# ssilverman16/particle_col_image_segmentation

Measured on AMD Instinct MI355X. Metric: Mpixels/sec segmented (5-ch 1024x1024 TIFF), ROI mask IoU=1.0, higher is better.
Workload: dtype f32 planes / u8 class maps / int32 labels / f64 ROI sums; 1 GPU; BASELINE config 2: batch of 64 frames 1024x1024x5 float32 per GPU, full kernel chain, inputs resident in HBM; frames_per_gpu=64, height=1024, width=1024, planes=5, parallelism=frames x1, launch=one hipGraph replay per step, 4 in flight, tie_fallback_frames_last_step=0, reference_nan_frames_rank0=0

## Files before the change

### particle_col_image_segmentation_amd/csrc/watershed.hip

```cpp
#include <algorithm>
#include <atomic>
#include <climits>
#include <mutex>
#include <type_traits>

#include "common.h"

namespace pcseg {

constexpr int WS_T = 64;
constexpr int WS_S = WS_T + 2;
constexpr int WS_P = 67;
constexpr int WS_N = WS_S * WS_P;
constexpr unsigned WS_INF = 0xFFFFFFFFu;
constexpr int WS_CNT0 = 32, WS_CNT_STRIDE = 32, WS_CHANGED_INTS = WS_CNT0 + 16 * WS_CNT_STRIDE;

__device__ __forceinline__ unsigned ws_key(float f)
{
    if (f == 0.0f) f = 0.0f;
    unsigned u = __float_as_uint(f);
    u = (u & 0x80000000u) ? ~u : (u | 0x80000000u);
    return u == WS_INF ? WS_INF - 1 : u;
}

__global__ void __launch_bounds__(256) ws_init_kernel(const float *__restrict__ img, int64_t frame_stride,
                                                       const int *__restrict__ markers, const uint8_t *__restrict__ mask,
                                                       unsigned *__restrict__ val, unsigned *__restrict__ L,
                                                       int *__restrict__ out, int64_t n, int64_t total)
{
    int64_t i = (int64_t)blockIdx.x * blockDim.x + threadIdx.x;
    if (i >= total) return;
    bool m = mask[i] != 0;
    unsigned v = m ? ws_key(img[(i / n) * frame_stride + (i % n)]) : WS_INF;
    int mk = m ? markers[i] : 0;
    val[i] = v;
    L[i] = mk != 0 ? v : WS_INF;
    out[i] = mk;
}

template <typename T>
__device__ __forceinline__ void ws_store_tile(const T *s, T *__restrict__ g, int r0, int c0, int H, int W)
{
    for (int i = threadIdx.x; i < WS_T * WS_T; i += blockDim.x) {
        int lr = i / WS_T, lc = i % WS_T;
        int r = r0 + lr, c = c0 + lc;
        if (r < H && c < W) g[rowoff(r, W) + c] = s[(lr + 1) * WS_P + lc + 1];
    }
}

template <typename T>
__device__ __forceinline__ void ws_mark_changed_edges(const T *s, const T *__restrict__ g, uint8_t *dirty_out,
                                                      int b, int tx, int ty, int tilesX, int tilesY, int r0, int c0, int H, int W)
{
    if (threadIdx.x >= 256) return;
    const int e = threadIdx.x >> 6, j = threadIdx.x & 63;
    const int lr = e == 0 ? 1 : (e == 1 ? WS_T : j + 1);
    const int lc = e == 2 ? 1 : (e == 3 ? WS_T : j + 1);
    const int r = r0 + lr - 1, c = c0 + lc - 1;
    bool ch = false;
    if (r < H && c < W) ch = s[lr * WS_P + lc] != g[rowoff(r, W) + c];
    if (__any(ch) && j == 0) {
        uint8_t *d = dirty_out + (int64_t)b * tilesX * tilesY;
        if (e == 0 && ty > 0) d[(ty - 1) * tilesX + tx] = 1;
        else if (e == 1 && ty + 1 < tilesY) d[(ty + 1) * tilesX + tx] = 1;
        else if (e == 2 && tx > 0) d[ty * tilesX + tx - 1] = 1;
        else if (e == 3 && tx + 1 < tilesX) d[ty * tilesX + tx + 1] = 1;
    }
}

template <int T>
struct RelaxGeom {
    static_assert(T == 64, "relaxation tiles are 64 pixels wide: one wave per sweep quadrant");
    static constexpr int S = T + 2;
    static constexpr int P = T + 4;
    static constexpr int PAD = 8;
    static constexpr int N = S * P + 2 * PAD;
    static constexpr int THREADS = 4 * 64;
    static constexpr int HE = T / 2;
    static constexpr size_t LDS_BYTES = sizeof(uint2) * N;
};

template <int DR, int DC, int P>
__device__ __forceinline__ bool ws_quadrant_sweep(uint2 *sLV, int lane)
{
    unsigned *sLw = reinterpret_cast<unsigned *>(sLV);
    typedef unsigned u2v __attribute__((ext_vector_type(2)));
    unsigned long long diff = 0;
    {
        constexpr int fr = DR > 0 ? 1 : WS_T, hr = DR > 0 ? 0 : WS_T + 1;
        const uint2 c = sLV[fr * P + 1 + lane];
        const unsigned h = sLV[hr * P + 1 + lane].x;
        const unsigned nw = min(c.x, max(c.y, h));
        atomicMin(&sLw[2 * (fr * P + 1 + lane)], nw);
        diff |= __ballot(nw != c.x);
    }
    const int lr = DR > 0 ? lane + 1 : WS_T - lane;
    const uint2 *row = sLV + lr * P;
    const unsigned halo = row[DC > 0 ? 0 : WS_T + 1].x;
    const int u0 = (0 - lane) & 63;
    unsigned left = row[DC > 0 ? u0 : WS_T + 1 - u0].x;
    const int un = (0 - (lane + 1)) & 63;
    unsigned prev = row[DC > 0 ? 1 + un : WS_T - un].x;
    const unsigned a0 = (unsigned)(uintptr_t)(row + (DC > 0 ? 1 : WS_T));
#pragma unroll 1
    for (int j0 = 0; j0 < WS_T; j0 += 8) {
        const int ub = (u0 + j0) & 63;
        const unsigned base_a = DC > 0 ? a0 + 8u * (unsigned)ub : a0 - 8u * (unsigned)ub - 56u;
        const unsigned base_b = DC > 0 ? base_a - 512u : base_a + 512u;
        unsigned ba[8];
        u2v t[8];
#define PCSEG_DS_READ(k)                                                                                                   \
        {                                                                                                                      \
            const unsigned long long wrapped = (((1ull << (k)) - 1ull) << 1) << j0;                \
            asm("v_cndmask_b32_e64 %0, %1, %2, %3" : "=v"(ba[k]) : "v"(base_a), "v"(base_b), "s"(wrapped));                     \
            asm volatile("ds_read_b64 %0, %1 offset:%2" : "=v"(t[k]) : "v"(ba[k]), "n"(DC > 0 ? 8 * (k) : 8 * (7 - (k))));     \
        }
        PCSEG_DS_READ(0) PCSEG_DS_READ(1) PCSEG_DS_READ(2) PCSEG_DS_READ(3)
        PCSEG_DS_READ(4) PCSEG_DS_READ(5) PCSEG_DS_READ(6) PCSEG_DS_READ(7)
#undef PCSEG_DS_READ
        asm volatile("s_waitcnt lgkmcnt(0)" : "+v"(t[0]), "+v"(t[1]), "+v"(t[2]), "+v"(t[3]), "+v"(t[4]), "+v"(t[5]), "+v"(t[6]), "+v"(t[7]));
        unsigned wr[8];
        unsigned long long batch_diff = 0;
#pragma unroll
        for (int k = 0; k < 8; ++k) {
            const unsigned up = (unsigned)__builtin_amdgcn_update_dpp((int)WS_INF, (int)prev, 0x138, 0xF, 0xF, false);
            const unsigned long long at0 = (1ull << k) << j0;
            unsigned lf;
            asm("v_cndmask_b32_e64 %0, %1, %2, %3" : "=v"(lf) : "v"(left), "v"(halo), "s"(at0));
            const unsigned cur = t[k].x, v = t[k].y;
            const unsigned m = min(up, lf);
            const unsigned cand = min(max(v, m), max(min(v, m), cur));
            wr[k] = cand;
            batch_diff |= __ballot(cur != cand);
            left = cand;
            prev = cand;
        }
        if (batch_diff != 0) {
#define PCSEG_DS_MIN(k)                                                                                                             \
            asm volatile("ds_min_u32 %0, %1 offset:%2" : : "v"(ba[k]), "v"(wr[k]), "n"(DC > 0 ? 8 * (k) : 8 * (7 - (k))) : "memory");
            PCSEG_DS_MIN(0) PCSEG_DS_MIN(1) PCSEG_DS_MIN(2) PCSEG_DS_MIN(3)
            PCSEG_DS_MIN(4) PCSEG_DS_MIN(5) PCSEG_DS_MIN(6) PCSEG_DS_MIN(7)
#undef PCSEG_DS_MIN
            diff |= batch_diff;
        }
    }
    return diff != 0;
}

struct WsInputs {
    const float *img;
    int64_t frame_stride;
    const int *markers;
    const uint8_t *mask;
    int *out;
    bool vec;
};

struct WsTiling {
    int off;
    int nx, ny;
};

template <int T>
__device__ __forceinline__ void ws_relax_tile(uint2 *sLV, const WsInputs &in, const bool FIRST, unsigned *__restrict__ val,
                                              unsigned *__restrict__ L, uint8_t *__restrict__ dirty_in,
                                              uint8_t *__restrict__ dirty_out, int *__restrict__ any_changed, int H, int W,
                                              const WsTiling &cur, const WsTiling &nxt, int max_iter, int tx, int ty, int b,
                                              int *__restrict__ list_out = nullptr, int *__restrict__ count_out = nullptr)
{
    using G = RelaxGeom<T>;
    constexpr int S = G::S, P = G::P, NT = G::THREADS, QW = T / 4;
    const int tid = threadIdx.x;
    if (!FIRST) {
        uint8_t *mark = dirty_in + ((int64_t)b * cur.ny + ty) * cur.nx + tx;
        if (!*mark) return;
        __syncthreads();
        if (tid == 0) *mark = 0;
    }
    if (tid == 0) atomicAdd(any_changed + WS_CNT0 + WS_CNT_STRIDE * ((tx + 5 * ty + 3 * b) & 15), 1);
    const int r0 = ty * T - cur.off, c0 = tx * T - cur.off;
    const int64_t fbase = (int64_t)b * H * W;
    auto initial = [&](int r, int c) -> uint2 {
        const int64_t g = fbase + rowoff(r, W) + c;
        if (!in.mask[g]) return make_uint2(WS_INF, WS_INF);
        const unsigned v = ws_key(in.img[(int64_t)b * in.frame_stride + rowoff(r, W) + c]);
        return make_uint2(in.markers[g] != 0 ? v : WS_INF, v);
    };
    if (in.vec) {
        constexpr int QUADS = S * QW, TRIPS = (QUADS + NT - 1) / NT;
        const float *img_f = in.img + (int64_t)b * in.frame_stride;
        const bool halo_thread = tid < 2 * S;
        const int h_lr = tid >> 1, h_lc = (tid & 1) ? S - 1 : 0;
        const int h_r = r0 + h_lr - 1, h_c = c0 + h_lc - 1;
        const bool h_in = halo_thread && h_r >= 0 && h_r < H && h_c >= 0 && h_c < W;
        const int64_t h_p = rowoff(min(max(h_r, 0), H - 1), W) + min(max(h_c, 0), W - 1);
        if (FIRST) {
            float4 f4[TRIPS];
            int4 m4[TRIPS];
            unsigned k4[TRIPS];
#pragma unroll
            for (int t = 0; t < TRIPS; ++t) {
                const int idx = min(tid + NT * t, QUADS - 1);
                const int lr = idx / QW, q = idx % QW;
                const int64_t p = rowoff(min(max(r0 + lr - 1, 0), H - 1), W) + min(max(c0 + 4 * q, 0), W - 4);
                f4[t] = *reinterpret_cast<const float4 *>(img_f + p);
                m4[t] = *reinterpret_cast<const int4 *>(in.markers + fbase + p);
                k4[t] = *reinterpret_cast<const unsigned *>(in.mask + fbase + p);
            }
            const float hf = img_f[h_p];
            const int hm = in.markers[fbase + h_p];
            const uint8_t hk = in.mask[fbase + h_p];
#pragma unroll
            for (int t = 0; t < TRIPS; ++t) {
                const int idx = tid + NT * t;
                if (idx < QUADS) {
                    const int lr = idx / QW, q = idx % QW;
                    const int r = r0 + lr - 1, c = c0 + 4 * q;
                    const bool inside = r >= 0 && r < H && c >= 0 && c < W;
                    const float fv[4] = {f4[t].x, f4[t].y, f4[t].z, f4[t].w};
                    const int mv[4] = {m4[t].x, m4[t].y, m4[t].z, m4[t].w};
                    unsigned key[4];
                    int lab[4];
#pragma unroll
                    for (int j = 0; j < 4; ++j) {
                        const bool msk = inside && ((k4[t] >> (8 * j)) & 255u) != 0;
                        key[j] = msk ? ws_key(fv[j]) : WS_INF;
                        lab[j] = msk ? mv[j] : 0;
                        sLV[lr * P + 1 + 4 * q + j] = make_uint2(lab[j] != 0 ? key[j] : WS_INF, key[j]);
                    }
                    if (inside && lr >= 1 && lr <= T) {
                        const int64_t g = fbase + rowoff(r, W) + c;
                        *reinterpret_cast<uint4 *>(val + g) = make_uint4(key[0], key[1], key[2], key[3]);
                        *reinterpret_cast<int4 *>(in.out + g) = make_int4(lab[0], lab[1], lab[2], lab[3]);
                    }
                }
            }
            if (halo_thread) {
                const bool msk = h_in && hk != 0;
                const unsigned key = msk ? ws_key(hf) : WS_INF;
                sLV[h_lr * P + h_lc] = make_uint2(msk && hm != 0 ? key : WS_INF, key);
            }
        } else {
            uint4 l4[TRIPS], v4[TRIPS];
#pragma unroll
            for (int t = 0; t < TRIPS; ++t) {
                const int idx = min(tid + NT * t, QUADS - 1);
                const int lr = idx / QW, q = idx % QW;
                const int64_t p = fbase + rowoff(min(max(r0 + lr - 1, 0), H - 1), W) + min(max(c0 + 4 * q, 0), W - 4);
                l4[t] = *reinterpret_cast<const uint4 *>(L + p);
                v4[t] = *reinterpret_cast<const uint4 *>(val + p);
            }
            const unsigned hl = L[fbase + h_p], hv = val[fbase + h_p];
#pragma unroll
            for (int t = 0; t < TRIPS; ++t) {
                const int idx = tid + NT * t;
                if (idx < QUADS) {
                    const int lr = idx / QW, q = idx % QW;
                    const int r = r0 + lr - 1, c = c0 + 4 * q;
                    const bool inside = r >= 0 && r < H && c >= 0 && c < W;
                    uint2 *dst = sLV + lr * P + 1 + 4 * q;
                    dst[0] = inside ? make_uint2(l4[t].x, v4[t].x) : make_uint2(WS_INF, WS_INF);
                    dst[1] = inside ? make_uint2(l4[t].y, v4[t].y) : make_uint2(WS_INF, WS_INF);
                    dst[2] = inside ? make_uint2(l4[t].z, v4[t].z) : make_uint2(WS_INF, WS_INF);
                    dst[3] = inside ? make_uint2(l4[t].w, v4[t].w) : make_uint2(WS_INF, WS_INF);
                }
            }
            if (halo_thread) sLV[h_lr * P + h_lc] = h_in ? make_uint2(hl, hv) : make_uint2(WS_INF, WS_INF);
        }
    } else
    for (int i = tid; i < S * S; i += NT) {
        int lr = i / S, lc = i % S;
        int r = r0 + lr - 1, c = c0 + lc - 1;
        uint2 lv = make_uint2(WS_INF, WS_INF);
        if (r >= 0 && r < H && c >= 0 && c < W) {
            if (FIRST) {
                lv = initial(r, c);
                if (lr >= 1 && lr <= T && lc >= 1 && lc <= T) {
                    const int64_t g = fbase + rowoff(r, W) + c;
                    val[g] = lv.y;
                    in.out[g] = lv.y != WS_INF ? in.markers[g] : 0;
                }
            } else {
                lv.x = L[fbase + rowoff(r, W) + c];
                lv.y = val[fbase + rowoff(r, W) + c];
            }
        }
        sLV[lr * P + lc] = lv;
    }
    __syncthreads();
    const bool rim_thread = tid < 8 * G::HE;
    const int e = tid / G::HE, ej = tid % G::HE;
    const int qy = e < 4 ? (e >> 1) : (e & 1), qx = e < 4 ? (e & 1) : ((e >> 1) & 1);
    const int rim_lr = e < 4 ? (qy ? T : 1) : qy * G::HE + ej + 1;
    const int rim_lc = e < 4 ? qx * G::HE + ej + 1 : (qx ? T : 1);
    const unsigned rim_before = rim_thread ? sLV[rim_lr * P + rim_lc].x : 0u;
    const int dir = (tid >> 6) & 3, lane = tid & 63;
    bool changed_any = false;
    bool capped = true;
    for (int iter = 0; iter < max_iter; ++iter) {
        bool changed;
        if (dir == 0) changed = ws_quadrant_sweep<1, 1, P>(sLV, lane);
        else if (dir == 1) changed = ws_quadrant_sweep<1, -1, P>(sLV, lane);
        else if (dir == 2) changed = ws_quadrant_sweep<-1, 1, P>(sLV, lane);
        else changed = ws_quadrant_sweep<-1, -1, P>(sLV, lane);
        if (!__syncthreads_or(changed)) { capped = false; break; }
        changed_any = true;
    }
    if (!FIRST && !changed_any) return;
    if (changed_any) {
        const int r = r0 + rim_lr - 1, c = c0 + rim_lc - 1;
        bool ch = rim_thread && capped;
        if (rim_thread && !capped && r >= 0 && r < H && c >= 0 && c < W) ch = sLV[rim_lr * P + rim_lc].x != rim_before;
        const unsigned long long mine = ((1ull << G::HE) - 1ull) << ((tid & 63) / G::HE * G::HE);
        const unsigned long long edge_changed = __ballot(ch) & mine;
        if (rim_thread && edge_changed && ej == 0) {
            const int oy = (r0 + qy * G::HE + nxt.off) / T, ox = (c0 + qx * G::HE + nxt.off) / T;
            if (oy >= 0 && oy < nxt.ny && ox >= 0 && ox < nxt.nx) {
                const int64_t m = ((int64_t)b * nxt.ny + oy) * nxt.nx + ox;
                if (list_out) {
                    const unsigned bit = 1u << (8 * (int)(m & 3));
                    const unsigned old = atomicOr(reinterpret_cast<unsigned *>(dirty_out + (m & ~(int64_t)3)), bit);
                    if (!(old & bit)) list_out[atomicAdd(count_out, 1)] = (int)m;
                } else {
                    dirty_out[m] = 1;
                }
            }
        }
    }
    __syncthreads();
    if (in.vec) {
#pragma unroll
        for (int t = 0; t < T * QW / NT; ++t) {
            const int idx = tid + NT * t, lr = idx / QW, q = idx % QW;
            const int r = r0 + lr, c = c0 + 4 * q;
            const uint2 *src = sLV + (lr + 1) * P + 1 + 4 * q;
            if (r >= 0 && r < H && c >= 0 && c < W)
                *reinterpret_cast<uint4 *>(L + fbase + rowoff(r, W) + c) = make_uint4(src[0].x, src[1].x, src[2].x, src[3].x);
        }
        return;
    }
    for (int i = tid; i < T * T; i += NT) {
        int lr = i / T, lc = i % T;
        int r = r0 + lr, c = c0 + lc;
        if (r >= 0 && r < H && c >= 0 && c < W) L[fbase + rowoff(r, W) + c] = sLV[(lr + 1) * P + lc + 1].x;
    }
}

template <int T>
__global__ void __launch_bounds__(RelaxGeom<T>::THREADS) ws_relax_kernel(WsInputs in, const bool FIRST, unsigned *__restrict__ val,
                                                                         unsigned *__restrict__ L, uint8_t *__restrict__ dirty_in,
                                                                         uint8_t *__restrict__ dirty_out, int *__restrict__ any_changed,
                                                                         int H, int W, WsTiling cur, WsTiling nxt, int max_iter,
                                                                         int *__restrict__ list_out, int *__restrict__ count_out)
{
    extern __shared__ __attribute__((aligned(16))) uint2 relax_lds[];
    const TileIndex t = xcd_tile_index();
    ws_relax_tile<T>(relax_lds + RelaxGeom<T>::PAD, in, FIRST, val, L, dirty_in, dirty_out, any_changed, H, W, cur, nxt, max_iter, t.x, t.y,
                     t.z, list_out, count_out);
}

constexpr int WS_LIST_FROM = 4, WS_LIST_GRID = 1024;

template <int T>
__global__ void __launch_bounds__(RelaxGeom<T>::THREADS) ws_relax_list_kernel(WsInputs in, unsigned *__restrict__ val, unsigned *__restrict__ L,
                                                                              uint8_t *__restrict__ dirty_in, uint8_t *__restrict__ dirty_out,
                                                                              int *__restrict__ any_changed, int H, int W, WsTiling cur,
                                                                              WsTiling nxt, int max_iter, const int *__restrict__ list_in,
                                                                              const int *__restrict__ count_in, int *__restrict__ list_out,
                                                                              int *__restrict__ count_out)
{
    extern __shared__ __attribute__((aligned(16))) uint2 relax_lds[];
    const int n = *count_in, per_frame = cur.nx * cur.ny;
    for (int i = blockIdx.x; i < n; i += gridDim.x) {
        const int m = list_in[i], b = m / per_frame, t = m % per_frame;
        ws_relax_tile<T>(relax_lds + RelaxGeom<T>::PAD, in, false, val, L, dirty_in, dirty_out, any_changed, H, W, cur, nxt, max_iter,
                         t % cur.nx, t / cur.nx, b, list_out, count_out);
        __syncthreads();
    }
}

constexpr int WS_TAIL_LIST = 1024;

template <int T>
__global__ void __launch_bounds__(RelaxGeom<T>::THREADS) ws_relax_tail_kernel(WsInputs in, unsigned *__restrict__ val,
                                                                              unsigned *__restrict__ L, uint8_t *__restrict__ dirtyA,
                                                                              uint8_t *__restrict__ dirtyB, int *__restrict__ any_changed,
                                                                              int *__restrict__ not_converged, int *__restrict__ exact_flags,
                                                                              int H, int W, WsTiling t0, WsTiling t1, int first_round,
                                                                              int max_rounds)
{
    extern __shared__ __attribute__((aligned(16))) uint2 relax_lds[];
    __shared__ int tail_list[WS_TAIL_LIST];
    __shared__ int tail_count;
    const int b = blockIdx.x;
    uint8_t *din = dirtyA, *dout = dirtyB;
    for (int round = first_round;; ++round) {
        const WsTiling cur = (round & 1) ? t1 : t0, nxt = (round & 1) ? t0 : t1;
        const int ntiles = cur.nx * cur.ny;
        const uint8_t *marks = din + (int64_t)b * ntiles;
        if (threadIdx.x == 0) tail_count = 0;
        __syncthreads();
        for (int t = threadIdx.x; t < ntiles; t += RelaxGeom<T>::THREADS)
            if (marks[t] != 0) {
                const int k = atomicAdd(&tail_count, 1);
                if (k < WS_TAIL_LIST) tail_list[k] = t;
            }
        __syncthreads();
        const int marked = tail_count;
        if (marked == 0) return;
        if (round - first_round >= max_rounds) {
            if (threadIdx.x == 0) { *not_converged = 1; exact_flags[b] = 1; }
            return;
        }
        const int walk = marked <= WS_TAIL_LIST ? marked : ntiles;
        for (int k = 0; k < walk; ++k) {
            const int t = marked <= WS_TAIL_LIST ? tail_list[k] : k;
            ws_relax_tile<T>(relax_lds + RelaxGeom<T>::PAD, in, false, val, L, din, dout, any_changed, H, W, cur, nxt, 100000, t % cur.nx,
                             t / cur.nx, b);
            __syncthreads();
        }
        uint8_t *tmp = din; din = dout; dout = tmp;
    }
}


constexpr int WS_LIST_SPAN = 8;
template <typename Body>
__device__ __forceinline__ void ws_for_frames(const int *frame_list, int grid_index, int grid_size, Body &&body)
{
    if (!frame_list) {
        body(grid_index);
        return;
    }
    const int n = frame_list[-1];
    for (int gi = grid_index; gi < n; gi += grid_size) body(frame_list[gi]);
}
static inline int ws_frame_span(const int *frame_list, int B) { return frame_list ? (B < WS_LIST_SPAN ? B : WS_LIST_SPAN) : B; }

__device__ __forceinline__ bool ws_active(const uint8_t *active, int b, int r, int c, int tilesX, int tilesY)
{
    return active == nullptr || active[((int64_t)b * tilesY + r / WS_T) * tilesX + c / WS_T] != 0;
}

struct WsTileList {
    const int *list;
    int ntpf, tilesX;
};
constexpr int WS_TILE_GRID = 512;

template <typename Body>
__device__ __forceinline__ void ws_for_tiles(const WsTileList &tl, Body &&body)
{
    const int n = tl.list[-1];
    for (int i = blockIdx.x; i < n; i += gridDim.x) {
        const int e = tl.list[i], b = e / tl.ntpf, t = e % tl.ntpf;
        body(b, t % tl.tilesX, t / tl.tilesX);
    }
}

__global__ void __launch_bounds__(256) ws_list_tiles_kernel(const int *__restrict__ frame_list, const uint8_t *__restrict__ active, int ntpf,
                                                             int *__restrict__ tile_list)
{
    ws_for_frames(frame_list, blockIdx.x, gridDim.x, [&](const int b) {
        for (int t = threadIdx.x; t < ntpf; t += 256)
            if (active[(int64_t)b * ntpf + t]) tile_list[atomicAdd(&tile_list[-1], 1)] = b * ntpf + t;
    });
}

constexpr int UF_TW = 64, UF_TH = 32, UF_SW = UF_TW + 2, UF_SH = UF_TH + 2;
constexpr int UF_LNS = UF_TW * UF_TH;
constexpr int UF_NS = 1 << 30;

__device__ __forceinline__ int vfind_lds(int *par, int v)
{
    int p;
    while ((p = ld_lds(par + (v & (UF_LNS - 1)))) != v) {
        const int g = ld_lds(par + (p & (UF_LNS - 1)));
        if (g != p) st_lds(par + (v & (UF_LNS - 1)), g);
        v = g;
    }
    return v;
}
__device__ __forceinline__ void vunite_lds(int *par, int a, int b)
{
    for (;;) {
        a = vfind_lds(par, a);
        b = vfind_lds(par, b);
        if (a == b) return;
        if (a < b) { int t = a; a = b; b = t; }
        int old = atomicMin(&par[a & (UF_LNS - 1)], b);
        if (old == a) return;
        a = old;
    }
}
__device__ __forceinline__ bool vwalk_ok(int x, int p, int n) { return (unsigned)p <= (unsigned)x && (p & (UF_NS - 1)) < n; }

__device__ __forceinline__ void vunite_glb(int *par, int p, int q, int n, int *corrupt)
{
    int a = ld_agent(par + p), b = ld_agent(par + q);
    bool ok = a >= 0 && b >= 0 && (a & (UF_NS - 1)) < n && (b & (UF_NS - 1)) < n;
    while (ok) {
        for (;;) {
            if (a == b) return;
            const int pa = ld_agent(par + (a & (UF_NS - 1))), pb = ld_agent(par + (b & (UF_NS - 1)));
            if (pa == a && pb == b) break;
            if (!vwalk_ok(a, pa, n) || !vwalk_ok(b, pb, n)) { ok = false; break; }
            const int ga = ld_agent(par + (pa & (UF_NS - 1))), gb = ld_agent(par + (pb & (UF_NS - 1)));
            if (!vwalk_ok(pa, ga, n) || !vwalk_ok(pb, gb, n)) { ok = false; break; }
            if (pa != a) {
                if (ga != pa) __hip_atomic_store(par + (a & (UF_NS - 1)), ga, __ATOMIC_RELAXED, __HIP_MEMORY_SCOPE_AGENT);
                a = ga;
            }
            if (pb != b) {
                if (gb != pb) __hip_atomic_store(par + (b & (UF_NS - 1)), gb, __ATOMIC_RELAXED, __HIP_MEMORY_SCOPE_AGENT);
                b = gb;
            }
        }
        if (!ok) break;
        if (a == b) return;
        if (a < b) { int t = a; a = b; b = t; }
        int old = atomicMin(par + (a & (UF_NS - 1)), b);
        if (old == a) return;
        if (!vwalk_ok(a, old, n)) break;
        a = old;
    }
    walk_corrupt(corrupt);
}
__device__ __forceinline__ int vwalk_root(const int *par, int x, int n, bool &bad)
{
    int q;
    while ((q = par[x & (UF_NS - 1)]) != x) {
        if (!vwalk_ok(x, q, n)) {
            bad = true;
            break;
        }
        x = q;
    }
    return x;
}

template <typename KeyT>
__device__ __forceinline__ void ws_uf_tile_frame(KeyT *sK, int *par, uint8_t *sM, const int b, const int tile_x, const int tile_y,
                                                 const KeyT *__restrict__ K,
                                                 const int *__restrict__ F, const uint8_t *__restrict__ active,
                                                 int *__restrict__ parent, uint8_t *__restrict__ minmask, uint8_t *__restrict__ bad,
                                                 int H, int W, int tilesX, int tilesY)
{
    const KeyT KINF = ~(KeyT)0;
    const int r0 = tile_y * UF_TH, c0 = tile_x * UF_TW;
    if (!ws_active(active, b, r0, c0, tilesX, tilesY)) return;
    const int64_t fbase = (int64_t)b * H * W;
    if (sizeof(KeyT) == 4 && (W & 3) == 0 && c0 + UF_TW <= W && (((uintptr_t)K) & 15) == 0) {
        constexpr int QUADS = UF_SH * (UF_TW / 4), TRIPS = (QUADS + 255) / 256;
        uint4 kq[TRIPS];
#pragma unroll
        for (int t = 0; t < TRIPS; ++t) {
            const int i = min((int)threadIdx.x + 256 * t, QUADS - 1);
            const int r = r0 + i / (UF_TW / 4) - 1;
            kq[t] = *reinterpret_cast<const uint4 *>(K + fbase + rowoff(min(max(r, 0), H - 1), W) + c0 + 4 * (i % (UF_TW / 4)));
        }
        const int hl = min((int)threadIdx.x, UF_SH * 2 - 1);
        const int hr = r0 + (hl >> 1) - 1, hx = (hl & 1) ? UF_TW : -1, hc = c0 + hx;
        const KeyT hv = K[fbase + rowoff(min(max(hr, 0), H - 1), W) + min(max(hc, 0), W - 1)];
#pragma unroll
        for (int t = 0; t < TRIPS; ++t) {
            const int i = (int)threadIdx.x + 256 * t;
            if (i < QUADS) {
                const int lr = i / (UF_TW / 4), r = r0 + lr - 1;
                const bool in = r >= 0 && r < H;
                KeyT *dst = sK + lr * UF_SW + 1 + 4 * (i % (UF_TW / 4));
                dst[0] = in ? (KeyT)kq[t].x : KINF; dst[1] = in ? (KeyT)kq[t].y : KINF;
                dst[2] = in ? (KeyT)kq[t].z : KINF; dst[3] = in ? (KeyT)kq[t].w : KINF;
            }
        }
        if (threadIdx.x < UF_SH * 2) sK[(hl >> 1) * UF_SW + hx + 1] = (hr >= 0 && hr < H && hc >= 0 && hc < W) ? hv : KINF;
    } else {
        constexpr int TRIPS = (UF_SH * UF_SW + 255) / 256;
        KeyT kv[TRIPS];
#pragma unroll
        for (int t = 0; t < TRIPS; ++t) {
            const int i = min((int)threadIdx.x + 256 * t, UF_SH * UF_SW - 1);
            const int r = r0 + i / UF_SW - 1, c = c0 + i % UF_SW - 1;
            kv[t] = K[fbase + rowoff(min(max(r, 0), H - 1), W) + min(max(c, 0), W - 1)];
        }
#pragma unroll
        for (int t = 0; t < TRIPS; ++t) {
            const int i = (int)threadIdx.x + 256 * t;
            const int r = r0 + i / UF_SW - 1, c = c0 + i % UF_SW - 1;
            if (i < UF_SH * UF_SW) sK[i] = (r >= 0 && r < H && c >= 0 && c < W) ? kv[t] : KINF;
        }
    }
    __syncthreads();
    int self[UF_LNS / 256];
    int fv[UF_LNS / 256];
#pragma unroll
    for (int k = 0; k < UF_LNS / 256; ++k) {
        const int t = threadIdx.x + k * 256;
        fv[k] = F[fbase + rowoff(min(r0 + t / UF_TW, H - 1), W) + min(c0 + t % UF_TW, W - 1)];
    }
#pragma unroll
    for (int k = 0; k < UF_LNS / 256; ++k) {
        const int t = threadIdx.x + k * 256;
        const int lr = t / UF_TW, lc = t % UF_TW;
        const int r = r0 + lr, c = c0 + lc;
        const int i = (lr + 1) * UF_SW + lc + 1;
        int v = -1;
        if ((unsigned)(sK[i] >> (8 * sizeof(KeyT) - 32)) != WS_INF)
            v = fv[k] != 0 ? t : t + UF_LNS;
        uint8_t m8 = 0;
        if (v >= UF_LNS) {
            const KeyT ku = sK[i - UF_SW], kl = sK[i - 1], kr = sK[i + 1], kd = sK[i + UF_SW];
            const KeyT m = min(min(ku, kd), min(kl, kr));
            if (m != KINF) m8 = (ku == m ? 1 : 0) | (kl == m ? 2 : 0) | (kr == m ? 4 : 0) | (kd == m ? 8 : 0);
        }
        self[k] = v;
        sM[t] = m8;
        if (r < H && c < W) {
            minmask[fbase + rowoff(r, W) + c] = m8;
            if (fv[k] != 0) bad[fbase + rowoff(r, W) + c] = 0;
        }
    }
    __syncthreads();
#pragma unroll
    for (int k = 0; k < UF_LNS / 256; ++k) {
        const int t = threadIdx.x + k * 256;
        const int lc = t % UF_TW;
        const bool joins_left = lc > 0 && ((sM[t] & 2) || (sM[t - 1] & 4));
        const unsigned long long heads = __ballot(!joins_left);
        const unsigned long long seeds = __ballot(self[k] >= 0 && self[k] < UF_LNS);
        const unsigned long long upto = heads & (lc == 63 ? ~0ull : ((2ull << lc) - 1ull));
        const int start = 63 - __clzll((long long)upto);
        const unsigned long long later = lc == 63 ? 0ull : (heads >> (lc + 1));
        const int end = later ? lc + (__ffsll((long long)later) - 1) : 63;
        const unsigned long long run = (end == 63 ? ~0ull : ((2ull << end) - 1ull)) & ~((1ull << start) - 1ull);
        const unsigned long long run_seeds = seeds & run;
        int root = -1;
        if (self[k] >= 0) {
            if (run_seeds) root = (t - lc) + (__ffsll((long long)run_seeds) - 1);
            else root = (t - lc) + start + UF_LNS;
        }
        par[t] = root;
    }
    __syncthreads();
#pragma unroll
    for (int k = 0; k < UF_LNS / 256; ++k) {
        const int t = threadIdx.x + k * 256;
        const int lr = t / UF_TW, lc = t % UF_TW;
        if (lr == 0 || self[k] < 0) continue;
        const uint8_t m = sM[t], mu = sM[t - UF_TW];
        if (!((m & 1) || (mu & 8))) continue;
        if (lc > 0) {
            const uint8_t ml = sM[t - 1], mul = sM[t - UF_TW - 1];
            const bool same_run = (m & 2) || (ml & 4), same_run_up = (mu & 2) || (mul & 4), left_vertical = (ml & 1) || (mul & 8);
            if (same_run && same_run_up && left_vertical) continue;
        }
        vunite_lds(par, par[t], par[t - UF_TW]);
    }
    __syncthreads();
    for (int t = threadIdx.x; t < UF_TH * UF_TW; t += 256) {
        const int r = r0 + t / UF_TW, c = c0 + t % UF_TW;
        if (r >= H || c >= W) continue;
        int v = -1;
        if (par[t] >= 0) {
            const int root = vfind_lds(par, par[t]);
            const int lt = root & (UF_LNS - 1);
            v = ((r0 + lt / UF_TW) * W + c0 + lt % UF_TW) | (root >= UF_LNS ? UF_NS : 0);
        }
        parent[fbase + rowoff(r, W) + c] = v;
    }
}

template <typename KeyT, bool LIST>
__global__ void __launch_bounds__(256) ws_uf_tile_kernel(WsTileList tiles, const KeyT *__restrict__ K, const int *__restrict__ F,
                                                          const uint8_t *__restrict__ active, int *__restrict__ parent,
                                                          uint8_t *__restrict__ minmask, uint8_t *__restrict__ bad, int H, int W,
                                                          int tilesX, int tilesY)
{
    __shared__ KeyT sK[UF_SH * UF_SW];
    __shared__ int par[UF_TH * UF_TW];
// ... 1138 lines not shown
```

Baseline: 16530 Mpixels/s.

## Prefetch next list tile into registers during relax sweep, tighten rim dirty marking

Splits the relax tile routine into load-issue, commit, sweep-and-mark and store phases. The list kernel now issues global loads for the next tile into registers before running the current tile's sweep, hiding load latency behind the sweep, and it adds a launch-bounds occupancy hint. The rim-change test now also requires the changed label to actually be able to propagate into the neighbour (max of neighbour value and new label below neighbour label), so fewer neighbour tiles get marked dirty. The register prefetch raises register pressure, and the stricter marking condition risks correctness if the propagation test is wrong. Profiling scripts are also added.

```diff
diff --git a/particle_col_image_segmentation_amd/csrc/watershed.hip b/particle_col_image_segmentation_amd/csrc/watershed.hip
--- a/particle_col_image_segmentation_amd/csrc/watershed.hip
+++ b/particle_col_image_segmentation_amd/csrc/watershed.hip
@@ -162,22 +162,78 @@
 };
 
 template <int T>
-__device__ __forceinline__ void ws_relax_tile(uint2 *sLV, const WsInputs &in, const bool FIRST, unsigned *__restrict__ val,
-                                              unsigned *__restrict__ L, uint8_t *__restrict__ dirty_in,
-                                              uint8_t *__restrict__ dirty_out, int *__restrict__ any_changed, int H, int W,
-                                              const WsTiling &cur, const WsTiling &nxt, int max_iter, int tx, int ty, int b,
-                                              int *__restrict__ list_out = nullptr, int *__restrict__ count_out = nullptr)
+struct WsTileRegs {
+    static constexpr int QW = T / 4, QUADS = RelaxGeom<T>::S * QW;
+    static constexpr int TRIPS = (QUADS + RelaxGeom<T>::THREADS - 1) / RelaxGeom<T>::THREADS;
+    uint4 l4[TRIPS], v4[TRIPS];
+    unsigned hl, hv;
+};
+
+template <int T>
+__device__ __forceinline__ void ws_tile_load_issue(WsTileRegs<T> &rg, const unsigned *__restrict__ val, const unsigned *__restrict__ L,
+                                                   int H, int W, const WsTiling &cur, int tx, int ty, int b)
+{
+    using G = RelaxGeom<T>;
+    using R = WsTileRegs<T>;
+    const int tid = threadIdx.x;
+    const int r0 = ty * T - cur.off, c0 = tx * T - cur.off;
+    const int64_t fbase = (int64_t)b * H * W;
+#pragma unroll
+    for (int t = 0; t < R::TRIPS; ++t) {
+        const int idx = min(tid + G::THREADS * t, R::QUADS - 1);
+        const int lr = idx / R::QW, q = idx % R::QW;
+        const int64_t p = fbase + rowoff(min(max(r0 + lr - 1, 0), H - 1), W) + min(max(c0 + 4 * q, 0), W - 4);
+        rg.l4[t] = *reinterpret_cast<const uint4 *>(L + p);
+        rg.v4[t] = *reinterpret_cast<const uint4 *>(val + p);
+    }
+    const int h_lr = min(tid >> 1, G::S - 1), h_lc = (tid & 1) ? G::S - 1 : 0;
+    const int64_t h_p = fbase + rowoff(min(max(r0 + h_lr - 1, 0), H - 1), W) + min(max(c0 + h_lc - 1, 0), W - 1);
+    rg.hl = L[h_p];
+    rg.hv = val[h_p];
+}
+
+template <int T>
+__device__ __forceinline__ void ws_tile_load_commit(uint2 *sLV, const WsTileRegs<T> &rg, int H, int W, const WsTiling &cur, int tx, int ty)
+{
+    using G = RelaxGeom<T>;
+    using R = WsTileRegs<T>;
+    constexpr int P = G::P;
+    const int tid = threadIdx.x;
+    const int r0 = ty * T - cur.off, c0 = tx * T - cur.off;
+    const uint2 out = make_uint2(WS_INF, WS_INF);
+#pragma unroll
+    for (int t = 0; t < R::TRIPS; ++t) {
+        const int idx = tid + G::THREADS * t;
+        if (idx < R::QUADS) {
+            const int lr = idx / R::QW, q = idx % R::QW;
+            const int r = r0 + lr - 1, c = c0 + 4 * q;
+            const bool inside = r >= 0 && r < H && c >= 0 && c < W;
+            uint2 *dst = sLV + lr * P + 1 + 4 * q;
+            dst[0] = inside ? make_uint2(rg.l4[t].x, rg.v4[t].x) : out;
+            dst[1] = inside ? make_uint2(rg.l4[t].y, rg.v4[t].y) : out;
+            dst[2] = inside ? make_uint2(rg.l4[t].z, rg.v4[t].z) : out;
+            dst[3] = inside ? make_uint2(rg.l4[t].w, rg.v4[t].w) : out;
+        }
+    }
+    if (tid < 2 * G::S) {
+        const int h_lr = tid >> 1, h_lc = (tid & 1) ? G::S - 1 : 0;
+        const int h_r = r0 + h_lr - 1, h_c = c0 + h_lc - 1;
+        sLV[h_lr * P + h_lc] = h_r >= 0 && h_r < H && h_c >= 0 && h_c < W ? make_uint2(rg.hl, rg.hv) : out;
+    }
+}
+
+__device__ __forceinline__ void ws_count_tile(int *__restrict__ any_changed, int tx, int ty, int b)
+{
+    if (threadIdx.x == 0) atomicAdd(any_changed + WS_CNT0 + WS_CNT_STRIDE * ((tx + 5 * ty + 3 * b) & 15), 1);
+}
+
+template <int T>
+__device__ __forceinline__ void ws_tile_load(uint2 *sLV, const WsInputs &in, const bool FIRST, unsigned *__restrict__ val,
+                                             const unsigned *__restrict__ L, int H, int W, const WsTiling &cur, int tx, int ty, int b)
 {
     using G = RelaxGeom<T>;
     constexpr int S = G::S, P = G::P, NT = G::THREADS, QW = T / 4;
     const int tid = threadIdx.x;
-    if (!FIRST) {
-        uint8_t *mark = dirty_in + ((int64_t)b * cur.ny + ty) * cur.nx + tx;
-        if (!*mark) return;
-        __syncthreads();
-        if (tid == 0) *mark = 0;
-    }
-    if (tid == 0) atomicAdd(any_changed + WS_CNT0 + WS_CNT_STRIDE * ((tx + 5 * ty + 3 * b) & 15), 1);
     const int r0 = ty * T - cur.off, c0 = tx * T - cur.off;
     const int64_t fbase = (int64_t)b * H * W;
     auto initial = [&](int r, int c) -> uint2 {
@@ -194,7 +250,11 @@
         const int h_r = r0 + h_lr - 1, h_c = c0 + h_lc - 1;
         const bool h_in = halo_thread && h_r >= 0 && h_r < H && h_c >= 0 && h_c < W;
         const int64_t h_p = rowoff(min(max(h_r, 0), H - 1), W) + min(max(h_c, 0), W - 1);
-        if (FIRST) {
+        if (!FIRST) {
+            WsTileRegs<T> rg;
+            ws_tile_load_issue<T>(rg, val, L, H, W, cur, tx, ty, b);
+            ws_tile_load_commit<T>(sLV, rg, H, W, cur, tx, ty);
+        } else {
             float4 f4[TRIPS];
             int4 m4[TRIPS];
             unsigned k4[TRIPS];
@@ -240,32 +300,6 @@
                 const unsigned key = msk ? ws_key(hf) : WS_INF;
                 sLV[h_lr * P + h_lc] = make_uint2(msk && hm != 0 ? key : WS_INF, key);
             }
-        } else {
-            uint4 l4[TRIPS], v4[TRIPS];
-#pragma unroll
-            for (int t = 0; t < TRIPS; ++t) {
-                const int idx = min(tid + NT * t, QUADS - 1);
-                const int lr = idx / QW, q = idx % QW;
-                const int64_t p = fbase + rowoff(min(max(r0 + lr - 1, 0), H - 1), W) + min(max(c0 + 4 * q, 0), W - 4);
-                l4[t] = *reinterpret_cast<const uint4 *>(L + p);
-                v4[t] = *reinterpret_cast<const uint4 *>(val + p);
-            }
-            const unsigned hl = L[fbase + h_p], hv = val[fbase + h_p];
-#pragma unroll
-            for (int t = 0; t < TRIPS; ++t) {
-                const int idx = tid + NT * t;
-                if (idx < QUADS) {
-                    const int lr = idx / QW, q = idx % QW;
-                    const int r = r0 + lr - 1, c = c0 + 4 * q;
-                    const bool inside = r >= 0 && r < H && c >= 0 && c < W;
-                    uint2 *dst = sLV + lr * P + 1 + 4 * q;
-                    dst[0] = inside ? make_uint2(l4[t].x, v4[t].x) : make_uint2(WS_INF, WS_INF);
-                    dst[1] = inside ? make_uint2(l4[t].y, v4[t].y) : make_uint2(WS_INF, WS_INF);
-                    dst[2] = inside ? make_uint2(l4[t].z, v4[t].z) : make_uint2(WS_INF, WS_INF);
-                    dst[3] = inside ? make_uint2(l4[t].w, v4[t].w) : make_uint2(WS_INF, WS_INF);
-                }
-            }
-            if (halo_thread) sLV[h_lr * P + h_lc] = h_in ? make_uint2(hl, hv) : make_uint2(WS_INF, WS_INF);
         }
     } else
     for (int i = tid; i < S * S; i += NT) {
@@ -287,7 +321,17 @@
         }
         sLV[lr * P + lc] = lv;
     }
-    __syncthreads();
+}
+
+template <int T>
+__device__ __forceinline__ bool ws_tile_sweep_and_mark(uint2 *sLV, const bool FIRST, uint8_t *__restrict__ dirty_out, int H, int W,
+                                                       const WsTiling &cur, const WsTiling &nxt, int max_iter, int tx, int ty, int b,
+                                                       int *__restrict__ list_out, int *__restrict__ count_out)
+{
+    using G = RelaxGeom<T>;
+    constexpr int P = G::P;
+    const int tid = threadIdx.x;
+    const int r0 = ty * T - cur.off, c0 = tx * T - cur.off;
     const bool rim_thread = tid < 8 * G::HE;
     const int e = tid / G::HE, ej = tid % G::HE;
     const int qy = e < 4 ? (e >> 1) : (e & 1), qx = e < 4 ? (e & 1) : ((e >> 1) & 1);
@@ -306,11 +350,15 @@
         if (!__syncthreads_or(changed)) { capped = false; break; }
         changed_any = true;
     }
-    if (!FIRST && !changed_any) return;
+    if (!FIRST && !changed_any) return false;
     if (changed_any) {
         const int r = r0 + rim_lr - 1, c = c0 + rim_lc - 1;
         bool ch = rim_thread && capped;
-        if (rim_thread && !capped && r >= 0 && r < H && c >= 0 && c < W) ch = sLV[rim_lr * P + rim_lc].x != rim_before;
+        if (rim_thread && !capped && r >= 0 && r < H && c >= 0 && c < W) {
+            const unsigned now = sLV[rim_lr * P + rim_lc].x;
+            const uint2 y = sLV[(e < 4 ? (qy ? T + 1 : 0) : rim_lr) * P + (e < 4 ? rim_lc : (qx ? T + 1 : 0))];
+            ch = now != rim_before && max(y.y, now) < y.x;
+        }
         const unsigned long long mine = ((1ull << G::HE) - 1ull) << ((tid & 63) / G::HE * G::HE);
         const unsigned long long edge_changed = __ballot(ch) & mine;
         if (rim_thread && edge_changed && ej == 0) {
@@ -327,7 +375,18 @@
             }
         }
     }
-    __syncthreads();
+    return true;
+}
+
+template <int T>
+__device__ __forceinline__ void ws_tile_store(const uint2 *sLV, const WsInputs &in, unsigned *__restrict__ L, int H, int W,
+                                              const WsTiling &cur, int tx, int ty, int b)
+{
+    using G = RelaxGeom<T>;
+    constexpr int P = G::P, NT = G::THREADS, QW = T / 4;
+    const int tid = threadIdx.x;
+    const int r0 = ty * T - cur.off, c0 = tx * T - cur.off;
+    const int64_t fbase = (int64_t)b * H * W;
     if (in.vec) {
 #pragma unroll
         for (int t = 0; t < T * QW / NT; ++t) {
@@ -347,6 +406,27 @@
 }
 
 template <int T>
+__device__ __forceinline__ void ws_relax_tile(uint2 *sLV, const WsInputs &in, const bool FIRST, unsigned *__restrict__ val,
+                                              unsigned *__restrict__ L, uint8_t *__restrict__ dirty_in,
+                                              uint8_t *__restrict__ dirty_out, int *__restrict__ any_changed, int H, int W,
+                                              const WsTiling &cur, const WsTiling &nxt, int max_iter, int tx, int ty, int b,
+                                              int *__restrict__ list_out = nullptr, int *__restrict__ count_out = nullptr)
+{
+    if (!FIRST) {
+        uint8_t *mark = dirty_in + ((int64_t)b * cur.ny + ty) * cur.nx + tx;
+        if (!*mark) return;
+        __syncthreads();
+        if (threadIdx.x == 0) *mark = 0;
+    }
+    ws_count_tile(any_changed, tx, ty, b);
+    ws_tile_load<T>(sLV, in, FIRST, val, L, H, W, cur, tx, ty, b);
+    __syncthreads();
+    if (!ws_tile_sweep_and_mark<T>(sLV, FIRST, dirty_out, H, W, cur, nxt, max_iter, tx, ty, b, list_out, count_out)) return;
+    __syncthreads();
+    ws_tile_store<T>(sLV, in, L, H, W, cur, tx, ty, b);
+}
+
+template <int T>
 __global__ void __launch_bounds__(RelaxGeom<T>::THREADS) ws_relax_kernel(WsInputs in, const bool FIRST, unsigned *__restrict__ val,
                                                                          unsigned *__restrict__ L, uint8_t *__restrict__ dirty_in,
                                                                          uint8_t *__restrict__ dirty_out, int *__restrict__ any_changed,
@@ -360,21 +440,48 @@
 }
 
 constexpr int WS_LIST_FROM = 4, WS_LIST_GRID = 1024;
-
 template <int T>
-__global__ void __launch_bounds__(RelaxGeom<T>::THREADS) ws_relax_list_kernel(WsInputs in, unsigned *__restrict__ val, unsigned *__restrict__ L,
-                                                                              uint8_t *__restrict__ dirty_in, uint8_t *__restrict__ dirty_out,
-                                                                              int *__restrict__ any_changed, int H, int W, WsTiling cur,
-                                                                              WsTiling nxt, int max_iter, const int *__restrict__ list_in,
-                                                                              const int *__restrict__ count_in, int *__restrict__ list_out,
-                                                                              int *__restrict__ count_out)
+__global__ void __launch_bounds__(RelaxGeom<T>::THREADS, 4) ws_relax_list_kernel(WsInputs in, unsigned *__restrict__ val, unsigned *__restrict__ L,
+                                                                                 uint8_t *__restrict__ dirty_in, uint8_t *__restrict__ dirty_out,
+                                                                                 int *__restrict__ any_changed, int H, int W, WsTiling cur,
+                                                                                 WsTiling nxt, int max_iter, const int *__restrict__ list_in,
+                                                                                 const int *__restrict__ count_in, int *__restrict__ list_out,
+                                                                                 int *__restrict__ count_out)
 {
     extern __shared__ __attribute__((aligned(16))) uint2 relax_lds[];
+    uint2 *sLV = relax_lds + RelaxGeom<T>::PAD;
     const int n = *count_in, per_frame = cur.nx * cur.ny;
-    for (int i = blockIdx.x; i < n; i += gridDim.x) {
-        const int m = list_in[i], b = m / per_frame, t = m % per_frame;
-        ws_relax_tile<T>(relax_lds + RelaxGeom<T>::PAD, in, false, val, L, dirty_in, dirty_out, any_changed, H, W, cur, nxt, max_iter,
-                         t % cur.nx, t / cur.nx, b, list_out, count_out);
+    int i = blockIdx.x;
+    if (i >= n) return;
+    if (!in.vec) {
+        for (; i < n; i += gridDim.x) {
+            const int m = list_in[i], b = m / per_frame, t = m % per_frame;
+            ws_relax_tile<T>(sLV, in, false, val, L, dirty_in, dirty_out, any_changed, H, W, cur, nxt, max_iter, t % cur.nx, t / cur.nx, b,
+                             list_out, count_out);
+            __syncthreads();
+        }
+        return;
+    }
+    WsTileRegs<T> rg;
+    int m = list_in[i], m_next = i + (int)gridDim.x < n ? list_in[i + gridDim.x] : 0;
+    ws_tile_load_issue<T>(rg, val, L, H, W, cur, (m % per_frame) % cur.nx, (m % per_frame) / cur.nx, m / per_frame);
+    for (;;) {
+        const int b = m / per_frame, t = m % per_frame, tx = t % cur.nx, ty = t / cur.nx;
+        if (threadIdx.x == 0) dirty_in[m] = 0;
+        ws_count_tile(any_changed, tx, ty, b);
+        ws_tile_load_commit<T>(sLV, rg, H, W, cur, tx, ty);
+        i += gridDim.x;
+        if (i < n) {
+            m = m_next;
+            ws_tile_load_issue<T>(rg, val, L, H, W, cur, (m % per_frame) % cur.nx, (m % per_frame) / cur.nx, m / per_frame);
+            if (i + (int)gridDim.x < n) m_next = list_in[i + gridDim.x];
+        }
+        __syncthreads();
+        if (ws_tile_sweep_and_mark<T>(sLV, false, dirty_out, H, W, cur, nxt, max_iter, tx, ty, b, list_out, count_out)) {
+            __syncthreads();
+            ws_tile_store<T>(sLV, in, L, H, W, cur, tx, ty, b);
+        }
+        if (i >= n) return;
         __syncthreads();
     }
 }
diff --git a/profiles/relax_walk/time_relax.py b/profiles/relax_walk/time_relax.py
--- /dev/null
+++ b/profiles/relax_walk/time_relax.py
@@ -0,0 +1,46 @@
+import ctypes
+import json
+import os
+import sys
+
+import torch
+
+sys.path.insert(0, os.path.join(os.path.dirname(os.path.abspath(__file__)), "..", ".."))
+from particle_col_image_segmentation_amd import _lib, synth
+from particle_col_image_segmentation_amd.pipeline import FramePipeline
+
+STEPS = int(sys.argv[1]) if len(sys.argv) > 1 else 6
+B, H, W = 64, 1024, 1024
+lib = _lib.load()
+dev = torch.device("cuda", 0)
+stack = synth.gen_batch_torch(10_000, B, H, W, dev)
+solo = FramePipeline(dict(synth.CELL_TYPES_5), overlap=False)
+for _ in range(2):
+    solo.run(stack)
+torch.cuda.synchronize()
+lib.pcseg_watershed_counters(None, 1)
+lib.pcseg_timing_enable(1)
+for _ in range(STEPS):
+    res = solo.run(stack)
+torch.cuda.synchronize()
+nbytes = lib.pcseg_timing_report(None, 0)
+buf = ctypes.create_string_buffer(nbytes + 16)
+lib.pcseg_timing_report(buf, nbytes + 16)
+lib.pcseg_timing_enable(0)
+cnt = (ctypes.c_int64 * 4)()
+lib.pcseg_watershed_counters(cnt, 0)
+kern = {}
+for line in buf.value.decode().splitlines():
+    name, calls, ms = line.split("\t")
+    kern[name.lstrip("(").split("<")[0].split("(")[0].strip()] = kern.get(name.lstrip("(").split("<")[0].split("(")[0].strip(), 0.0) + float(ms)
+out = {k: round(v / STEPS, 4) for k, v in kern.items() if k.startswith("ws_relax")}
+out["relax_ms_per_step"] = round(sum(v for k, v in kern.items() if k.startswith("ws_relax")) / STEPS, 4)
+out["ws_ms_per_step"] = round(sum(v for k, v in kern.items() if k.startswith("ws_")) / STEPS, 4)
+out["serial_kernel_ms_per_step"] = round(sum(kern.values()) / STEPS, 4)
+calls = max(int(cnt[2]), 1)
+out["tile_visits_per_call"] = round(int(cnt[0]) / calls, 1)
+out["relax_launches_per_call"] = round(int(cnt[1]) / calls, 2)
+out["watershed_calls"] = int(cnt[2])
+out["tie_frames"] = int(res["tie_flags"].sum().item())
+out["lib"] = os.environ.get("PCSEG_LIB", "in-tree")
+print(json.dumps(out))
diff --git a/profiles/relax_walk/trace_driver.py b/profiles/relax_walk/trace_driver.py
--- /dev/null
+++ b/profiles/relax_walk/trace_driver.py
@@ -0,0 +1,14 @@
+import os
+import sys
+
+import torch
+
+sys.path.insert(0, os.path.join(os.path.dirname(os.path.abspath(__file__)), "..", ".."))
+from particle_col_image_segmentation_amd import synth
+from particle_col_image_segmentation_amd.pipeline import FramePipeline
+
+stack = synth.gen_batch_torch(10_000, 64, 1024, 1024, torch.device("cuda", 0))
+solo = FramePipeline(dict(synth.CELL_TYPES_5), overlap=False)
+for _ in range(5):
+    solo.run(stack)
+torch.cuda.synchronize()
```

New measurement: 7122 Mpixels/s. -56.9%, worse.
